# huster-wgm/SRCGAN

Measured on AMD Instinct MI355X. Metric: paired SR-CycleGAN train images/sec at x4 256->1024, higher is better.
Workload: dtype bf16; 1 GPU; Sat2Aerx4 paired G+D step (BASELINE configs[1]): 23-block RRDB generator + 3-layer PatchGAN, 3x256x256->3x1024x1024, batch 16/GPU; per_gpu_batch=16, global_batch=16, parallelism=dp1, gradient_exchange=none (1 rank)

## Files before the change

include/srcgan_amd.h:

```cpp
#ifndef SRCGAN_AMD_H
#define SRCGAN_AMD_H

#include <stddef.h>
#include <stdint.h>

#ifdef __cplusplus
extern "C" {
#endif

#define SRCGAN_F32 0
#define SRCGAN_BF16 1
#define SRCGAN_F16 2

int srcgan_version(void);
const char* srcgan_last_error(void);
int srcgan_dtype_size(int dtype);

int srcgan_nchw_f32_to_nhwc(const float* src, void* dst, int B, int C, int H, int W,
                            int cs, int dtype, void* stream);
int srcgan_nhwc_to_nchw_f32(const void* src, float* dst, int B, int C, int H, int W,
                            int cs, int coff, int dtype, void* stream);

size_t srcgan_packed_weight_bytes(int rows, int kdim, int ntaps, int dtype);
int srcgan_pack_weight(const float* w, void* wp, int rows, int kdim, int tys, int txs,
                       long sr, long sk, long sty, long stx, long off, int dtype, void* stream);
int srcgan_pack_weight_part(const float* w, void* wp, int rows, int kdim, int tys, int txs,
                            long sr, long sk, long sty, long stx, long off, int k_off, int k_total, float scale,
                            int dtype, void* stream);

typedef struct srcgan_conv_desc {
    const void* x; const void* wp; const float* bias; void* y;
    const void* r1; const void* r2; const void* mz;
    int dtype;
    int kh, kw, stride;
    int B, H, W, Cin, x_cs, x_coff;
    int OH, OW, Cout;
    int YH, YW, y_cs, y_coff;
    int pad_y, pad_x, os, oa, ob;
    int r1_cs, r1_coff, r1_cend;
    int r2_cs, r2_coff, r2_cend;
    int mz_cs, mz_coff, mz_c0;
    float alpha, beta1, beta2, slope, mslope;
    int act;
    long x_plane, y_plane, r1_plane, r2_plane, mz_plane;
    int rev_batch;
    void* sign_out; const void* sign_in;
    int npar; long wpar_stride;
} srcgan_conv_desc;
int srcgan_conv_igemm(const srcgan_conv_desc* d, void* stream);

typedef struct srcgan_wgrad_desc {
    const void* dy; const void* x; float* slab; float* grad;
    float* bias_grad;
    int dtype;
    int kh, kw, stride;
    int B, H, W, Cin, x_cs, x_coff;
    int OH, OW, Cout, dy_cs, dy_coff;
    int pad_y, pad_x;
    int nsplit;
    long sr, sk, sty, stx, off;
    float alpha;
    int accumulate;
} srcgan_wgrad_desc;
size_t srcgan_conv_wgrad_slab_bytes(int Cout, int Cin, int kh, int kw, int nsplit);
int srcgan_conv_wgrad_nsplit(int B, int OH, int OW, int Cout, int Cin, int stride);
int srcgan_conv_wgrad(const srcgan_wgrad_desc* d, void* stream);

typedef struct srcgan_wgrad_seg { int g0, g1; float* grad; float* bias; int Cin; float alpha; } srcgan_wgrad_seg;
typedef struct srcgan_wgrad_dense_desc {
    const void* dy; const void* x; float* slab;
    int dtype;
    int B, H, W;
    int G, dy_cs, dy_coff;
    int C, x_cs, x_coff;
    int nseg;
    srcgan_wgrad_seg seg[8];
    int accumulate;
    long dy_plane, x_plane;
} srcgan_wgrad_dense_desc;
size_t srcgan_wgrad_dense_slab_bytes(int G, int C, int dtype, int B, int H, int W);
int srcgan_wgrad_dense(const srcgan_wgrad_dense_desc* d, void* stream);

// ... 404 lines not shown
```

srcgan_amd/_native.py:

```python
from __future__ import annotations

import ctypes as C
import os
from typing import Optional, Sequence

import torch

_HERE = os.path.dirname(os.path.abspath(__file__))
LIB_PATH = os.environ.get("SRCGAN_AMD_LIB") or os.path.join(_HERE, "lib", "libsrcgan_amd.so")

F32, BF16, F16 = 0, 1, 2
_DTYPES = {"fp32": F32, "f32": F32, "float32": F32, torch.float32: F32,
           "bf16": BF16, "bfloat16": BF16, torch.bfloat16: BF16,
           "fp16": F16, "f16": F16, "float16": F16, "half": F16, torch.float16: F16, F32: F32, BF16: BF16, F16: F16}
_default_dtype = _DTYPES[os.environ.get("SRCGAN_AMD_DTYPE", "fp32")]


def dtype_id(d) -> int:
    if d is None:
        return _default_dtype
    try:
        return _DTYPES[d]
    except KeyError:
        raise ValueError(f"unsupported compute dtype {d!r} (use 'fp32', 'bf16' or 'fp16')") from None
# ... 88 lines not shown

class VdsrCfg(C.Structure):
    _fields_ = [(n, C.c_int) for n in ("in_ch", "B", "H", "W", "dtype", "n_resblocks", "n_feats")]


class ResnetGenCfg(C.Structure):
    _fields_ = [(n, C.c_int) for n in ("in_ch", "out_ch", "B", "H", "W", "dtype", "ngf", "n_blocks", "padding")]


class UnetCfg(C.Structure):
    _fields_ = [(n, C.c_int) for n in ("in_ch", "out_ch", "B", "H", "W", "dtype", "ngf", "num_downs")]


class VggLossCfg(C.Structure):
    _fields_ = [(n, C.c_int) for n in ("kind", "B", "H", "W", "dtype")]


class NLayerDCfg(C.Structure):
    _fields_ = [("in_ch", C.c_int), ("ndf", C.c_int), ("n_layers", C.c_int),
                ("B", C.c_int), ("H", C.c_int), ("W", C.c_int), ("dtype", C.c_int), ("training", C.c_int), ("norm", C.c_int)]


_P, _I, _L, _F, _S = C.c_void_p, C.c_int, C.c_long, C.c_float, C.c_size_t
SIGNATURES = {
    "srcgan_version": (_I, []),
    "srcgan_last_error": (C.c_char_p, []),
    "srcgan_dtype_size": (_I, [_I]),
    "srcgan_nchw_f32_to_nhwc": (_I, [_P, _P, _I, _I, _I, _I, _I, _I, _P]),
    "srcgan_nhwc_to_nchw_f32": (_I, [_P, _P, _I, _I, _I, _I, _I, _I, _I, _P]),
    "srcgan_packed_weight_bytes": (_S, [_I, _I, _I, _I]),
    "srcgan_pack_weight": (_I, [_P, _P, _I, _I, _I, _I, _L, _L, _L, _L, _L, _I, _P]),
    "srcgan_pack_weight_part": (_I, [_P, _P, _I, _I, _I, _I, _L, _L, _L, _L, _L, _I, _I, _F, _I, _P]),
    "srcgan_conv_igemm": (_I, [C.POINTER(ConvDesc), _P]),
    "srcgan_conv_wgrad_slab_bytes": (_S, [_I, _I, _I, _I, _I]),
    "srcgan_conv_wgrad_nsplit": (_I, [_I, _I, _I, _I, _I, _I]),
    "srcgan_conv_wgrad": (_I, [C.POINTER(WgradDesc), _P]),
    "srcgan_wgrad_dense_slab_bytes": (_S, [_I, _I, _I, _I, _I, _I]),
    "srcgan_wgrad_dense": (_I, [C.POINTER(WgradDenseDesc), _P]),
    "srcgan_col_reduce_blocks": (_I, [_L]),
    "srcgan_col_reduce": (_I, [_I, _P, _I, _I, _P, _I, _I, _P, _P, _L, _I, _F, _P, _P, _P, _I, _P]),
    "srcgan_bn_finalize": (_I, [_P, _P, _P, _P, _P, _P, _I, _L, _F, _F, _P]),
    "srcgan_bn_eval_rstd": (_I, [_P, _P, _I, _F, _P]),
    "srcgan_bn_apply_lrelu": (_I, [_P, _P, _P, _P, _P, _P, _L, _I, _I, _F, _I, _P]),
    "srcgan_bn_bwd_apply": (_I, [_P, _P, _P, _P, _P, _P, _P, _P, _L, _I, _I, _I, _P]),
    "srcgan_add_inplace": (_I, [_P, _I, _I, _P, _I, _I, _P, _I, _I, _F, _L, _I, _I, _P]),
    "srcgan_add_inplace_planes": (_I, [_P, _I, _I, _L, _P, _I, _I, _L, _P, _I, _I, _L, _F, _L, _I, _I, _P]),
    "srcgan_gn_scratch_floats": (_S, [_I, _I]),
    "srcgan_gn_forward": (_I, [_P, _I, _P, _I, _P, _I, _P, _P, _P, _I, _L, _I, _I, _F, _I, _F, _I, _P, _P]),
    "srcgan_gn_backward": (_I, [_P, _I, _P, _I, _P, _I, _P, _P, _P, _I, _P, _I, _I, _P, _P, _I, _F, _I, _L, _I, _I, _I, _P, _P]),
    "srcgan_ca_scratch_floats": (_S, [_I, _L, _I]),
    "srcgan_ca_forward": (_I, [_P, _I, _P, _I, _P, _I, _P, _P, _P, _P, _P, _I, _L, _I, _I, _I, _P, _P]),
    "srcgan_ca_backward": (_I, [_P, _I, _P, _I, _P, _P, _P, _P, _I, _P, _I, _I, _P, _P, _P, _P, _I, _L, _I, _I, _I, _P, _P]),
    "srcgan_s2d_shift": (_I, [_P, _I, _P, _I, _I, _I, _I, _I, _I, _I, _I, _I, _I, _P]),
    "srcgan_d2s_shift": (_I, [_P, _I, _P, _I, _I, _I, _I, _I, _I, _I, _I, _I, _I, _I, _P]),
    "srcgan_prelu_forward": (_I, [_P, _I, _P, _P, _P, _I, _F, _P, _I, _I, _I, _I, _I, _I, _I, _I, _I, _I, _P]),
    "srcgan_prelu_scratch_floats": (_S, [_I, _I, _I, _I, _I]),
    "srcgan_prelu_backward": (_I, [_P, _I, _P, _I, _P, _P, _P, _I, _P, _I, _F, _I, _P, _P, _I, _I, _I, _I, _I, _I, _I, _I, _I, _P, _P]),
    "srcgan_reflect_pad_nhwc": (_I, [_P, _I, _P, _I, _I, _I, _I, _I, _I, _I, _P]),
    "srcgan_reflect_pad_bwd_nhwc": (_I, [_P, _I, _P, _I, _I, _I, _I, _I, _I, _I, _I, _P]),
    "srcgan_tanh_forward": (_I, [_P, _I, _P, _I, _L, _I, _I, _P]),
    "srcgan_tanh_backward": (_I, [_P, _I, _P, _I, _P, _I, _L, _I, _I, _I, _P]),
    "srcgan_in_skip_forward": (_I, [_P, _I, _P, _I, _P, _I, _I, _P, _I, _L, _I, _F, _F, _I, _P, _P]),
    "srcgan_relu_nhwc": (_I, [_P, _I, _P, _I, _I, _L, _I, _I, _P]),
    "srcgan_upsample2_nhwc": (_I, [_P, _I, _I, _L, _P, _I, _I, _I, _I, _I, _I, _P]),
    "srcgan_sum2x2_nhwc": (_I, [_P, _I, _P, _I, _P, _I, _F, _I, _I, _I, _I, _I, _P]),
    "srcgan_loss_scratch_floats": (_I, []),
# ... 190 lines not shown
```

srcgan_amd/build.py:

```python
import glob
import os
import subprocess
import sys
from concurrent.futures import ThreadPoolExecutor

HERE = os.path.dirname(os.path.abspath(__file__))
CSRC = os.path.join(HERE, "csrc")
LIBDIR = os.path.join(HERE, "lib")
LIB = os.path.join(LIBDIR, "libsrcgan_amd.so")
SOURCES = ["conv_entry.hip", "conv_igemm.hip", "conv_par4.hip", "deconv_k3s2.hip", "conv3x3_dma.hip", "conv_wgrad.hip", "wgrad_dense.hip", "elementwise.hip", "class_losses.hip", "groupnorm.hip", "chan_attn.hip", "back_proj.hip", "reflect_pad.hip", "unet_skip.hip", "metrics.hip", "shift_select.hip", "scene_score.hip", "colour.hip", "tiles.hip", "vgg_loss.hip", "nets.hip", "oplist.hip"]
FLAGS = ["--offload-arch=gfx950", "-O3", "-std=c++17", "-fPIC", "-Wall", "-Wno-unused-function"]


def _hipcc():
    for c in (os.environ.get("HIPCC"), "/opt/rocm/bin/hipcc", "hipcc"):
        if c and (os.path.isabs(c) and os.path.exists(c) or not os.path.isabs(c)):
            return c
    raise RuntimeError("hipcc not found")


def _stale(target, deps):
    if not os.path.exists(target):
        return True
    t = os.path.getmtime(target)
    return any(os.path.getmtime(d) > t for d in deps)


def build(force=False, verbose=True):
    os.makedirs(LIBDIR, exist_ok=True)
    hipcc = _hipcc()
    headers = glob.glob(os.path.join(CSRC, "*.h")) + [os.path.join(HERE, "..", "include", "srcgan_amd.h")]
    objs, jobs = [], []
    for s in SOURCES:
        src = os.path.join(CSRC, s)
        obj = os.path.join(LIBDIR, s.replace(".hip", ".o"))
        objs.append(obj)
        if force or _stale(obj, [src] + headers):
            jobs.append([hipcc, *FLAGS, "-c", src, "-o", obj])

    def run(cmd):
        if verbose:
            print("[srcgan_amd.build]", " ".join(cmd), flush=True)
        subprocess.run(cmd, check=True)
# ... 13 lines not shown
```

srcgan_amd/csrc/conv_entry.hip:

```cpp
#include "conv_params.h"

static const bool g_force_generic = sg_env("SRCGAN_GENERIC_3X3") != nullptr;

static int check_desc(const srcgan_conv_desc* d) {
    SG_REQUIRE(d && d->x && d->wp && d->y, "srcgan_conv_igemm: null pointer");
    SG_REQUIRE(sg_dtype_ok(d->dtype), "srcgan_conv_igemm: bad dtype %d", d->dtype);
    const int epp = d->dtype == SRCGAN_F32 ? 4 : 8;
    SG_REQUIRE(d->B > 0 && d->H > 0 && d->W > 0 && d->OH > 0 && d->OW > 0 && d->Cin > 0 && d->Cout > 0,
               "srcgan_conv_igemm: non-positive dimension");
    SG_REQUIRE(d->Cin % epp == 0 && d->x_cs % epp == 0 && d->x_coff % epp == 0,
               "srcgan_conv_igemm: input channels/stride/offset (%d,%d,%d) must be multiples of %d", d->Cin, d->x_cs, d->x_coff, epp);
    SG_REQUIRE((d->x_plane || d->x_coff + d->Cin <= d->x_cs) && (d->y_plane || d->y_coff + d->Cout <= d->y_cs),
               "srcgan_conv_igemm: channel slice exceeds stride");
    SG_REQUIRE(!d->x_plane || (d->kh == 3 && d->kw == 3 && d->stride == 1), "srcgan_conv_igemm: a blocked-layout input is supported by the 3x3 stride-1 kernel only");
    SG_REQUIRE(((uintptr_t)d->x % 16) == 0 && ((uintptr_t)d->wp % 16) == 0, "srcgan_conv_igemm: x/wp must be 16-byte aligned");
    SG_REQUIRE(d->os >= 1 && d->oa >= 0 && d->ob >= 0 && d->oa < d->os && d->ob < d->os, "srcgan_conv_igemm: bad output scale/offset");
    SG_REQUIRE((d->OH - 1) * d->os + d->oa < d->YH && (d->OW - 1) * d->os + d->ob < d->YW, "srcgan_conv_igemm: output extent exceeds tensor");
    if (d->sign_out || d->sign_in) {
        const bool dense32 = d->kh == 3 && d->kw == 3 && d->stride == 1 && sg_is16(d->dtype) && d->Cout == 32 && d->os == 1 && d->oa == 0 && d->ob == 0 &&
                             d->YH == d->OH && d->YW == d->OW && d->x_plane && !(d->sign_in && d->mz) && (!d->sign_out || d->act);
        const bool up_out = d->sign_out && !d->sign_in && d->kh == 1 && d->kw == 1 && d->npar == 4 && sg_is16(d->dtype) && d->Cout == 64 && d->act;
        const bool in64 = d->sign_in && !d->sign_out && d->kh == 3 && d->kw == 3 && d->stride == 1 && sg_is16(d->dtype) && d->Cout == 64 && d->os == 1 &&
                          d->YH == d->OH && d->YW == d->OW && !d->mz && !d->r1 && !d->r2;
        SG_REQUIRE(dense32 || up_out || in64,
// ... 46 lines not shown
               "3x3 stride-1 form (pad 1, whole 64-byte input chunks, 18 rows below 2 GiB) takes larger images", p.H, p.W, p.xpix);
    return 0;
}

static int route(const srcgan_conv_desc* d, ConvP& p, hipStream_t st) {
    if (d->npar && d->kh == 3) {
        SG_REQUIRE(d->npar == 4 && d->kw == 3 && d->stride == 2 && d->pad_y == 1 && d->pad_x == 1 && d->os == 2 && d->oa == 0 && d->ob == 0 &&
                   d->OH == d->H && d->OW == d->W && d->YH == 2 * d->H && d->YW == 2 * d->W && d->wpar_stride > 0 && d->wpar_stride % 16 == 0 &&
                   !d->x_plane && !d->y_plane && !d->sign_in && !d->sign_out,
                   "srcgan_conv_igemm: npar == 4 with a 3x3 kernel is the transposed stride-2 form: stride 2, pad 1, os 2, oa == ob == 0, OH x OW = H x W, "
                   "YH x YW = 2H x 2W, the four parity packs wpar_stride bytes apart, interleaved tensors, no sign masks");
        SG_TRY(sg_require_image_31(p));
        p.npar = 4; p.wpar = d->wpar_stride;
        return sg_deconv_k3s2(p, d->dtype, st);
    }
    if (d->npar && d->kh == 1 && d->kw == 1) {
        SG_REQUIRE(d->npar == 4 && d->stride == 1 && d->os == 2 && d->oa == 0 && d->ob == 0 && d->wpar_stride > 0 && d->wpar_stride % 16 == 0 &&
                   !d->sign_in, "srcgan_conv_igemm: npar == 4 with a 1x1 kernel needs os == 2, oa == ob == 0 and the four packs wpar_stride bytes apart");
        SG_REQUIRE(!d->sign_out || p.buf16, "srcgan_conv_igemm: sign_out of the 1x1 four-parity form needs 16-byte accessible output channels");
        p.npar = 4; p.wpar = d->wpar_stride;
    } else if (d->npar) {
        SG_REQUIRE(d->npar == 4 && d->kh == 2 && d->kw == 2 && d->stride == 1 && d->wpar_stride > 0 && d->wpar_stride % 16 == 0 && !d->x_plane && !d->y_plane &&
                   !d->sign_in && !d->sign_out,
                   "srcgan_conv_igemm: npar must be 0 or 4 (2x2 stride-1 parity packs wpar_stride bytes apart, interleaved tensors, no bias / sign masks)");
        SG_TRY(sg_require_image_31(p));
        p.wpar = d->wpar_stride;
        return sg_dgrad_s2k4(p, d->dtype, st);
    }
    if (d->kh == 3 && d->kw == 3 && d->stride == 1 && (!g_force_generic || d->x_plane)) return sg_conv3x3_dma(p, d->dtype, st);
    SG_TRY(sg_require_image_31(p));
    return sg_conv_generic(p, d->dtype, d->kh, d->kw, d->stride, st);
}

extern "C" int srcgan_conv_igemm(const srcgan_conv_desc* d, void* stream) {
    SG_TRY(check_desc(d));
    ConvP p = build_params(d);
    return route(d, p, (hipStream_t)stream);
}
```

srcgan_amd/csrc/conv_igemm.hip:

```cpp
#include "conv_epilogue.h"
#include "launch.h"
#include <type_traits>

#if defined(SG_DIAG) && defined(SG_IG_DIAG)
#define IG_DBG(p, bit) ((p).dbg & (bit))
#else
#define IG_DBG(p, bit) 0
#endif


template <typename T, int KH, int KW, int S, int MT, int PT, bool WPK>
__global__ __launch_bounds__(256) void conv_igemm_k(const ConvP p) {
    using D = DT<T>;
    constexpr int TH = 4 * PT, TW = 32;
    constexpr int IHT = (TH - 1) * S + KH, IWT = (TW - 1) * S + KW;
    constexpr int COT = 32 * MT, NTAP = KH * KW, PIXB = 80;
    constexpr int WROWS = (WPK ? KW : NTAP) * COT;
    constexpr int NPH = IHT * IWT * 4;
    constexpr int NPW = WROWS * 4;
    constexpr int HIT = (NPH + 255) / 256, WIT = (NPW + 255) / 256;
    extern __shared__ __attribute__((aligned(16))) char smem[];
    char* lds_h = smem;
    char* lds_w = smem + IHT * IWT * PIXB;

// ... 253 lines not shown
#define SG_CASE(KH_, KW_, S_, PT_, WPK_) \
    if (kh == KH_ && kw == KW_ && s == S_) return launch_igemm<T, KH_, KW_, S_, MT, PT_, WPK_>(p, ctiles, st);
    SG_CASE(3, 3, 1, 2, false)
    SG_CASE(1, 1, 1, 2, false)
    SG_CASE(2, 2, 2, 1, false)
#ifndef SG_PT22
#define SG_PT22 2
#endif
    SG_CASE(2, 2, 1, SG_PT22, false)
    SG_CASE(1, 2, 1, 2, false)
    SG_CASE(2, 1, 1, 2, false)
    SG_CASE(4, 4, 2, 1, true)
    SG_CASE(4, 4, 1, 2, true)
    SG_CASE(3, 4, 1, 2, true)
    SG_CASE(4, 3, 1, 2, true)
    SG_CASE(3, 3, 2, 1, false)
    SG_CASE(7, 7, 2, 1, true)
    SG_CASE(1, 1, 2, 2, false)
    SG_CASE(5, 5, 1, 2, true)
    SG_CASE(9, 9, 1, 2, true)
    SG_CASE(7, 7, 1, 2, true)
#undef SG_CASE
    SG_FAIL("srcgan_conv_igemm: unsupported kernel %dx%d stride %d", kh, kw, s);
}

int sg_conv_generic(const ConvP& p, int dtype, int kh, int kw, int stride, hipStream_t st) {
    if (p.npar == 4 && kh == 1 && kw == 1 && sg_is16(dtype) && p.Cout == 64 && p.ypix == 128 && p.ycoff == 0 && p.yplane == 64 && p.YW == 2 * p.OW &&
        p.buf16 && !p.bias && !p.r1 && !p.r2 && !p.mz && p.Cin % 32 == 0) {
        ConvP q = p;
        q.npar = 2; q.wpar = 2 * p.wpar; q.wsplit = p.wpar;
        q.Cout = 128; q.ypix *= 2; q.YW = p.YW / 2; q.osx = 1;
        return sg_dtype_dispatch16(dtype, [&](auto t) { return launch_igemm<decltype(t), 1, 1, 1, 4, SG_UP_PT, false>(q, 2, st); });
    }
    const int npm = p.npar ? p.npar : 1;
    if (p.Cout <= 32) return sg_dtype_dispatch(dtype, [&](auto t) { return dispatch_shape<decltype(t), 1>(p, kh, kw, stride, npm, st); });
#ifdef SG_MT4_22
    if (dtype == SRCGAN_BF16 && kh == 2 && kw == 2 && stride == 1 && p.Cout % 128 == 0)
        return launch_igemm<__bf16, 2, 2, 1, 4, SG_PT22, false>(p, p.Cout / 128, st);
#endif
    const int ctiles = cdiv(p.Cout, 64) * npm;
    return sg_dtype_dispatch(dtype, [&](auto t) { return dispatch_shape<decltype(t), 2>(p, kh, kw, stride, ctiles, st); });
}
```

srcgan_amd/csrc/conv_par4.hip:

```cpp
#include "conv_epilogue.h"
#include "launch.h"
#include <type_traits>

template <typename T, int PT, bool VEC16>
__global__ __launch_bounds__(256, 2) void dgrad_s2k4_k(const ConvP p) {
    using D = DT<T>;
    constexpr int TH = 4 * PT, TW = 32, IHT = TH + 2, IWT = TW + 2;
    constexpr int COT = 32, PIXB = 80, NPAR = 4, WROWS = 16 * COT;
    constexpr int NPH = IHT * IWT * 4, NPW = WROWS * 4;
    constexpr int HIT = (NPH + 255) / 256, WIT = NPW / 256;
    static_assert(NPW % 256 == 0, "weight pieces per thread");
    extern __shared__ __attribute__((aligned(16))) char smem[];
    char* lds_h = smem;
    char* lds_w = smem + IHT * IWT * PIXB;

    const int tid = threadIdx.x, lane = tid & 63, wave = tid >> 6, r = lane & 31, h = lane >> 5;
    int L;
    {
        const int nblk = gridDim.x, bid = blockIdx.x, xcd = bid & 7, q8 = nblk >> 3, r8 = nblk & 7;
        L = (xcd < r8 ? xcd * (q8 + 1) : r8 * (q8 + 1) + (xcd - r8) * q8) + (bid >> 3);
    }
    const int ct = L % p.ctiles;
    int t = L / p.ctiles;
    const int tx = t % p.tiles_x; t /= p.tiles_x;
// ... 91 lines not shown
        pq.OH = (p.YH - pq.oa + 1) / 2; pq.OW = (p.YW - pq.ob + 1) / 2;
        if constexpr (VEC16) {
#pragma unroll
            for (int q = 0; q < PT; ++q) conv_epilogue_lds_row<T, 1, PT>(pq, acc[par], q, lw, b, ct, t0 + wave * PT + q, u0, lane);
        } else
            conv_epilogue<T, 1, PT>(pq, acc[par], b, ct, t0 + wave * PT, u0, r, h);
    }
}

template <typename T, int PT, bool VEC16>
static int launch_par4v(const ConvP& p, hipStream_t st) {
    constexpr int TH = 4 * PT, IHT = TH + 2, IWT = 34;
    constexpr size_t STAGE = (size_t)IHT * IWT * 80 + (size_t)16 * 32 * 80, EPI = (size_t)4 * 32 * (32 * 4 + 16);
    constexpr size_t SMEM = STAGE > EPI ? STAGE : EPI;
    constexpr auto kern = dgrad_s2k4_k<T, PT, VEC16>;
    int dev = 0;
    SG_TRY(sg_current_device(dev));
    SG_TRY(sg_allow_lds<kern>(SMEM, dev));
    ConvP q = p;
    q.tiles_x = cdiv((p.YW + 1) / 2, 32);
    q.tiles_y = cdiv((p.YH + 1) / 2, TH);
    q.ctiles = cdiv(p.Cout, 32);
    dim3 grid((unsigned)((size_t)q.tiles_x * q.tiles_y * p.B * q.ctiles), 1, 1);
    char cls[96];
    snprintf(cls, sizeof(cls), "dgrad_s2k4<%s,4 parities>", sg_dtype_tag<T>());
    const double px = (double)p.B * p.YH * p.YW;
    const int tok = sg_prof_start(cls, 2.0 * px * 4 * p.Cin * p.Cout, ((double)p.B * p.H * p.W * p.Cin + px * p.Cout) * sizeof(T), st);
    hipLaunchKernelGGL(kern, grid, dim3(256), SMEM, st, q);
    sg_prof_stop(tok, st);
    SG_LAUNCH_CHECK();
    return 0;
}

template <typename T, int PT>
static int launch_par4(const ConvP& p, hipStream_t st) {
    SG_REQUIRE(p.buf16, "srcgan_conv_igemm: npar == 4 needs output / mask channels, strides and offsets that are multiples of 16 bytes (and channel planes below 2 GiB)");
    return launch_par4v<T, PT, true>(p, st);
}

#ifndef SG_P4PT
#define SG_P4PT 2
#endif
int sg_dgrad_s2k4(const ConvP& p, int dtype, hipStream_t st) {
    return sg_dtype_dispatch(dtype, [&](auto t) { return launch_par4<decltype(t), SG_P4PT>(p, st); });
}
```

srcgan_amd/csrc/conv_params.h:

```cpp
#pragma once
#include "common.h"

struct ConvP {
    const void* x; const void* wp; const float* bias; void* y;
    const void* r1; const void* r2; const void* mz;
    int B, H, W, Cin, xcoff;
    int OH, OW, Cout, YH, YW, ycoff;
    int pad_y, pad_x, os, oa, ob;
    int r1coff, r1cend, r2coff, r2cend, mzcoff, mzc0;
    long xpix, xplane, ypix, yplane, r1pix, r1plane, r2pix, r2plane, mzpix, mzplane;
    float alpha, beta1, beta2, slope, mslope;
    int act, vec, nchunk, tiles_x, tiles_y, ctiles;
    int vec16;
    int buf16;
    int rev;
    long wpar;
    int npar;
    int osx;
    long wsplit;
    unsigned char* sgn_out; const unsigned char* sgn_in;
    int dbg;
    unsigned long long* trace;
};

template <typename T>
__device__ __forceinline__ size_t chan_off(int c, long plane) {
    constexpr int KCE = DT<T>::KCE;
    return (size_t)(c / KCE) * plane + (size_t)(c % KCE) * sizeof(T);
}

int sg_conv3x3_dma(const ConvP& p, int dtype, hipStream_t st);
int sg_dgrad_s2k4(const ConvP& p, int dtype, hipStream_t st);
int sg_deconv_k3s2(const ConvP& p, int dtype, hipStream_t st);
int sg_conv_generic(const ConvP& p, int dtype, int kh, int kw, int stride, hipStream_t st);
int sg_require_image_31(const ConvP& p);
```

srcgan_amd/ops.py:

```python
from __future__ import annotations

import ctypes as C
from typing import Optional, Tuple

import torch

from . import _native as N

TORCH_DT = {N.F32: torch.float32, N.BF16: torch.bfloat16, N.F16: torch.float16}


def to_nhwc(x: torch.Tensor, cs: Optional[int] = None, dtype=None) -> torch.Tensor:
    N.require_cuda(x, "to_nhwc")
    dt = N.dtype_id(dtype)
    x = x.contiguous().float()
    B, Cc, H, W = x.shape
    cs = cs or Cc
    out = torch.empty(B, H, W, cs, dtype=TORCH_DT[dt], device=x.device)
    N.check(N.lib().srcgan_nchw_f32_to_nhwc(x.data_ptr(), out.data_ptr(), B, Cc, H, W, cs, dt, N.stream_ptr(x.device)), "to_nhwc")
    return out


def to_nchw(x: torch.Tensor, Cc: Optional[int] = None, coff: int = 0) -> torch.Tensor:
    N.require_cuda(x, "to_nchw")
# ... 22 lines not shown
    return xb.permute(1, 2, 3, 0, 4).reshape(B, H, W, npl * kce)[..., :Cc].contiguous()


def pack_weight(w: torch.Tensor, rows: int, kdim: int, tys: int, txs: int, sr: int, sk: int, sty: int, stx: int,
                off: int = 0, dtype=None) -> torch.Tensor:
    N.require_cuda(w, "pack_weight")
    dt = N.dtype_id(dtype)
    lib = N.lib()
    nbytes = lib.srcgan_packed_weight_bytes(rows, kdim, tys * txs, dt)
    out = torch.empty(nbytes, dtype=torch.uint8, device=w.device)
    N.check(lib.srcgan_pack_weight(w.contiguous().data_ptr(), out.data_ptr(), rows, kdim, tys, txs, sr, sk, sty, stx, off, dt,
                                   N.stream_ptr(w.device)), "pack_weight")
    return out


def pack_conv2d_fwd(w: torch.Tensor, dtype=None) -> torch.Tensor:
    co, ci, kh, kw = w.shape
    return pack_weight(w, co, ci, kh, kw, ci * kh * kw, kh * kw, kw, 1, 0, dtype)


def pack_conv2d_dgrad_s1(w: torch.Tensor, dtype=None) -> torch.Tensor:
    co, ci, kh, kw = w.shape
    return pack_weight(w, ci, co, kh, kw, kh * kw, ci * kh * kw, -kw, -1, kh * kw - 1, dtype)


def conv_igemm(x: torch.Tensor, wp: torch.Tensor, y: torch.Tensor, *, kh: int, kw: int, stride: int = 1, Cin: Optional[int] = None,
               x_coff: int = 0, Cout: int, y_coff: int = 0, OH: Optional[int] = None, OW: Optional[int] = None,
               pad: Tuple[int, int] = (0, 0), bias: Optional[torch.Tensor] = None, alpha: float = 1.0, act: bool = False,
               slope: float = 0.2, r1: Optional[torch.Tensor] = None, r1_coff: int = 0, r1_cend: int = 0, beta1: float = 0.0,
               r2: Optional[torch.Tensor] = None, r2_coff: int = 0, r2_cend: int = 0, beta2: float = 0.0,
               mz: Optional[torch.Tensor] = None, mz_coff: int = 0, mz_c0: int = 0, mslope: float = 0.2,
               os: int = 1, oa: int = 0, ob: int = 0, x_plane: int = 0, y_plane: int = 0, r1_plane: int = 0, r2_plane: int = 0,
               mz_plane: int = 0, shape: Optional[Tuple[int, int, int]] = None, sign_out: Optional[torch.Tensor] = None,
               sign_in: Optional[torch.Tensor] = None, npar: int = 0, wpar_stride: int = 0, rev_batch: int = 0) -> torch.Tensor:
    N.require_cuda(x, "conv_igemm")
    d = N.ConvDesc()
    if shape is not None:
        (B, H, W), xcs = shape, x.shape[-1]
    else:
        B, H, W, xcs = x.shape
    d.x, d.wp, d.y = x.data_ptr(), wp.data_ptr(), y.data_ptr()
    d.bias = bias.data_ptr() if bias is not None else None
    d.dtype = N.dtype_id(x.dtype)
    d.kh, d.kw, d.stride = kh, kw, stride
    d.B, d.H, d.W, d.Cin, d.x_cs, d.x_coff = B, H, W, Cin or (xcs - x_coff), xcs, x_coff
    if OH is None:
        OH = (H + 2 * pad[0] - kh) // stride + 1
        OW = (W + 2 * pad[1] - kw) // stride + 1
    d.OH, d.OW, d.Cout = OH, OW, Cout
    d.YH, d.YW, d.y_cs, d.y_coff = (y.shape[-3], y.shape[-2], y.shape[-1], y_coff)
    d.pad_y, d.pad_x, d.os, d.oa, d.ob = pad[0], pad[1], os, oa, ob
    if r1 is not None:
        d.r1, d.r1_cs, d.r1_coff, d.r1_cend, d.beta1 = r1.data_ptr(), r1.shape[-1], r1_coff, r1_cend, beta1
    if r2 is not None:
        d.r2, d.r2_cs, d.r2_coff, d.r2_cend, d.beta2 = r2.data_ptr(), r2.shape[-1], r2_coff, r2_cend, beta2
    if mz is not None:
        d.mz, d.mz_cs, d.mz_coff, d.mz_c0 = mz.data_ptr(), mz.shape[-1], mz_coff, mz_c0
    if sign_out is not None:
        d.sign_out = sign_out.data_ptr()
    if sign_in is not None:
        d.sign_in = sign_in.data_ptr()
    d.npar, d.wpar_stride = npar, wpar_stride
    d.alpha, d.slope, d.mslope, d.act = alpha, slope, mslope, int(act)
    d.x_plane, d.y_plane, d.r1_plane, d.r2_plane, d.mz_plane = x_plane, y_plane, r1_plane, r2_plane, mz_plane
    d.rev_batch = rev_batch
    N.check(N.lib().srcgan_conv_igemm(C.byref(d), N.stream_ptr(x.device)), "srcgan_conv_igemm")
    return y


def pack_deconv3x3s2(w: torch.Tensor, dtype=None):
    N.require_cuda(w, "pack_deconv3x3s2")
    lib = N.lib()
    dt = N.dtype_id(dtype)
    cin, cout = w.shape[:2]
    w = w.contiguous().float()
    step = lib.srcgan_packed_weight_bytes(cout, cin, 4, dt)
    wp = torch.zeros(4 * step, dtype=torch.uint8, device=w.device)
    for q in range(4):
        a, b = q >> 1, q & 1
        N.check(lib.srcgan_pack_weight(w.data_ptr(), wp.data_ptr() + q * step, cout, cin, a + 1, b + 1, 9, cout * 9, -6, -2,
                                       (2 if a else 1) * 3 + (2 if b else 1), dt, N.stream_ptr(w.device)), "srcgan_pack_weight")
    return wp, step


def deconv3x3s2(x: torch.Tensor, w: torch.Tensor, bias: Optional[torch.Tensor] = None, relu: bool = False, packed=None,
                y: Optional[torch.Tensor] = None) -> torch.Tensor:
    N.require_cuda(x, "deconv3x3s2")
    B, H, W, _ = x.shape
    cout = w.shape[1]
    wp, step = packed if packed is not None else pack_deconv3x3s2(w, x.dtype)
    if y is None:
        y = torch.empty(B, 2 * H, 2 * W, cout, dtype=x.dtype, device=x.device)
    return conv_igemm(x, wp, y, kh=3, kw=3, stride=2, Cout=cout, OH=H, OW=W, pad=(1, 1), bias=bias, act=relu, slope=0.0, os=2,
                      npar=4, wpar_stride=step)


def conv_wgrad(dy: torch.Tensor, x: torch.Tensor, grad: torch.Tensor, *, kh: int, kw: int, stride: int = 1, Cout: int, Cin: int,
               dy_coff: int = 0, x_coff: int = 0, pad: Tuple[int, int] = (0, 0), layout: Tuple[int, int, int, int, int],
               alpha: float = 1.0, nsplit: Optional[int] = None, accumulate: bool = False,
               bias_grad: Optional[torch.Tensor] = None) -> torch.Tensor:
# ... 158 lines not shown
```

Baseline: 120.3 images/s.

## Add LDS-staged tiled kernels for 4x4 stride-2 conv and its parity dgrad

Adds a new persistent kernel for 4x4 stride-2 pad-1 convolutions in 16-bit types. It stages an 8x32 output tile's input halo and weights into LDS using async global-to-LDS loads with double buffering, and uses XCD-aware work distribution. It also adds a similar tiled kernel for the 4-parity 2x2 dgrad (the transpose of the stride-2 conv) that reuses one 3x3 input window across all parities. Both are meant to replace the generic igemm path for the PatchGAN downsampling layers and their backward passes, improving data reuse and overlapping loads with MFMA. A path-query API is added so callers can see which kernel a descriptor selects.

```diff
diff --git a/include/srcgan_amd.h b/include/srcgan_amd.h
--- a/include/srcgan_amd.h
+++ b/include/srcgan_amd.h
@@ -48,6 +48,7 @@
     int npar; long wpar_stride;
 } srcgan_conv_desc;
 int srcgan_conv_igemm(const srcgan_conv_desc* d, void* stream);
+int srcgan_conv_path(const srcgan_conv_desc* d);
 
 typedef struct srcgan_wgrad_desc {
     const void* dy; const void* x; float* slab; float* grad;
diff --git a/srcgan_amd/_native.py b/srcgan_amd/_native.py
--- a/srcgan_amd/_native.py
+++ b/srcgan_amd/_native.py
@@ -144,6 +144,7 @@
     "srcgan_pack_weight": (_I, [_P, _P, _I, _I, _I, _I, _L, _L, _L, _L, _L, _I, _P]),
     "srcgan_pack_weight_part": (_I, [_P, _P, _I, _I, _I, _I, _L, _L, _L, _L, _L, _I, _I, _F, _I, _P]),
     "srcgan_conv_igemm": (_I, [C.POINTER(ConvDesc), _P]),
+    "srcgan_conv_path": (_I, [C.POINTER(ConvDesc)]),
     "srcgan_conv_wgrad_slab_bytes": (_S, [_I, _I, _I, _I, _I]),
     "srcgan_conv_wgrad_nsplit": (_I, [_I, _I, _I, _I, _I, _I]),
     "srcgan_conv_wgrad": (_I, [C.POINTER(WgradDesc), _P]),
diff --git a/srcgan_amd/build.py b/srcgan_amd/build.py
--- a/srcgan_amd/build.py
+++ b/srcgan_amd/build.py
@@ -8,7 +8,7 @@
 CSRC = os.path.join(HERE, "csrc")
 LIBDIR = os.path.join(HERE, "lib")
 LIB = os.path.join(LIBDIR, "libsrcgan_amd.so")
-SOURCES = ["conv_entry.hip", "conv_igemm.hip", "conv_par4.hip", "deconv_k3s2.hip", "conv3x3_dma.hip", "conv_wgrad.hip", "wgrad_dense.hip", "elementwise.hip", "class_losses.hip", "groupnorm.hip", "chan_attn.hip", "back_proj.hip", "reflect_pad.hip", "unet_skip.hip", "metrics.hip", "shift_select.hip", "scene_score.hip", "colour.hip", "tiles.hip", "vgg_loss.hip", "nets.hip", "oplist.hip"]
+SOURCES = ["conv_entry.hip", "conv_igemm.hip", "conv_s2_tile8.hip", "conv_par4.hip", "deconv_k3s2.hip", "conv3x3_dma.hip", "conv_wgrad.hip", "wgrad_dense.hip", "elementwise.hip", "class_losses.hip", "groupnorm.hip", "chan_attn.hip", "back_proj.hip", "reflect_pad.hip", "unet_skip.hip", "metrics.hip", "shift_select.hip", "scene_score.hip", "colour.hip", "tiles.hip", "vgg_loss.hip", "nets.hip", "oplist.hip"]
 FLAGS = ["--offload-arch=gfx950", "-O3", "-std=c++17", "-fPIC", "-Wall", "-Wno-unused-function"]
 
 
diff --git a/srcgan_amd/csrc/conv_entry.hip b/srcgan_amd/csrc/conv_entry.hip
--- a/srcgan_amd/csrc/conv_entry.hip
+++ b/srcgan_amd/csrc/conv_entry.hip
@@ -102,6 +102,16 @@
     return sg_conv_generic(p, d->dtype, d->kh, d->kw, d->stride, st);
 }
 
+extern "C" int srcgan_conv_path(const srcgan_conv_desc* d) {
+    if (check_desc(d)) return -1;
+    const ConvP p = build_params(d);
+    if (d->npar == 4 && d->kh == 2 && d->kw == 2 && d->stride == 1 && d->wpar_stride > 0 && d->wpar_stride % 16 == 0 && !d->x_plane && !d->y_plane &&
+        !d->sign_in && !d->sign_out)
+        return sg_dgrad_s2k4_tile64_ok(p, d->dtype) ? 2 : 0;
+    const bool generic = !d->npar && !(d->kh == 3 && d->kw == 3 && d->stride == 1);
+    return generic && sg_conv_s2_tile8_ok(p, d->dtype, d->kh, d->kw, d->stride) ? 1 : 0;
+}
+
 extern "C" int srcgan_conv_igemm(const srcgan_conv_desc* d, void* stream) {
     SG_TRY(check_desc(d));
     ConvP p = build_params(d);
diff --git a/srcgan_amd/csrc/conv_igemm.hip b/srcgan_amd/csrc/conv_igemm.hip
--- a/srcgan_amd/csrc/conv_igemm.hip
+++ b/srcgan_amd/csrc/conv_igemm.hip
@@ -309,6 +309,7 @@
         q.Cout = 128; q.ypix *= 2; q.YW = p.YW / 2; q.osx = 1;
         return sg_dtype_dispatch16(dtype, [&](auto t) { return launch_igemm<decltype(t), 1, 1, 1, 4, SG_UP_PT, false>(q, 2, st); });
     }
+    if (sg_conv_s2_tile8_ok(p, dtype, kh, kw, stride)) return sg_conv_s2_tile8(p, dtype, st);
     const int npm = p.npar ? p.npar : 1;
     if (p.Cout <= 32) return sg_dtype_dispatch(dtype, [&](auto t) { return dispatch_shape<decltype(t), 1>(p, kh, kw, stride, npm, st); });
 #ifdef SG_MT4_22
diff --git a/srcgan_amd/csrc/conv_par4.hip b/srcgan_amd/csrc/conv_par4.hip
--- a/srcgan_amd/csrc/conv_par4.hip
+++ b/srcgan_amd/csrc/conv_par4.hip
@@ -147,6 +147,164 @@
     return 0;
 }
 
+static __device__ __attribute__((aligned(64))) unsigned int sg_p4_zero_page[16];
+typedef const __attribute__((address_space(1))) void* p4_gptr_t;
+typedef __attribute__((address_space(3))) void* p4_lptr_t;
+
+namespace p4t {
+constexpr int NWV = 8, TH = 8, TW = 32, IHT = TH + 2, IWT = TW + 2, COT = 64, REC = 32;
+constexpr int NHP = IHT * IWT;
+constexpr int HPIECES = (NHP * REC + 1023) / 1024, WPIECES = 16 * COT * REC / 1024;
+constexpr int HBYTES = HPIECES * 1024, WBYTES = WPIECES * 1024, SBYTES = HBYTES + WBYTES;
+constexpr int HIT = (HPIECES + NWV - 1) / NWV, WIT = WPIECES / NWV;
+constexpr int ERS = 32 * 4 + 16;
+constexpr size_t SMEM = 2 * (size_t)SBYTES;
+static_assert(WIT == 4, "weight piece `it` of a wave belongs to parity `it`: 8 pieces = 256 records per parity");
+static_assert(NWV * 32 * ERS <= SBYTES, "epilogue transpose space must fit one stage");
+__device__ __forceinline__ int half_off(int rec, int half) { return (half ^ ((rec >> 3) & 1)) * 16; }
+}
+
+template <typename T>
+__global__ __launch_bounds__(p4t::NWV * 64) void dgrad_s2k4_tile64_k(const ConvP p) {
+    using namespace p4t;
+    extern __shared__ __attribute__((aligned(1024))) char smem[];
+    const int tid = threadIdx.x, lane = tid & 63, r = lane & 31, h = lane >> 5;
+    const int wave = __builtin_amdgcn_readfirstlane(tid >> 6);
+    const int rp = wave & 3, mt = wave >> 2;
+    const int nunits = p.tiles_x * p.tiles_y * p.B * p.ctiles;
+    const int xcd = blockIdx.x & 7, jw = blockIdx.x >> 3, gw = (gridDim.x + 7 - xcd) >> 3;
+    const int u8 = (nunits + 7) >> 3;
+    const int u_lo = xcd * u8, u_hi = (u_lo + u8 < nunits) ? u_lo + u8 : nunits;
+    const char* zp = (const char*)sg_p4_zero_page;
+    const int nhalf = 2 * p.nchunk;
+
+    int w_off[WIT];
+#pragma unroll
+    for (int it = 0; it < WIT; ++it) {
+        const int q = (it * NWV + wave) * 64 + lane, rec = q >> 1;
+        w_off[it] = (rec & 255) * 64 + half_off(rec, q & 1);
+    }
+    int h_goff[HIT];
+    const char* f_xb = nullptr; const char* f_wb = nullptr;
+    auto setup_fetch = [&](int u, int& ob, int& oct, int& ot0, int& ou0) {
+        const int ct = u % p.ctiles; int t = u / p.ctiles;
+        const int tx = t % p.tiles_x; t /= p.tiles_x;
+        const int ty = t % p.tiles_y; const int b = t / p.tiles_y;
+        ob = b; oct = ct; ot0 = ty * TH; ou0 = tx * TW;
+        f_xb = (const char*)p.x + (size_t)b * p.H * p.W * p.xpix + (size_t)p.xcoff * sizeof(T);
+        f_wb = (const char*)p.wp + (size_t)ct * p.nchunk * 4 * COT * 64;
+#pragma unroll
+        for (int it = 0; it < HIT; ++it) {
+            const int q = (it * NWV + wave) * 64 + lane, rec = q >> 1;
+            const int iy = rec / IWT, ix = rec - iy * IWT;
+            const int gy = ot0 - 1 + iy, gx = ou0 - 1 + ix;
+            const bool ok = rec < NHP && (unsigned)gy < (unsigned)p.H && (unsigned)gx < (unsigned)p.W;
+            h_goff[it] = ok ? (gy * p.W + gx) * (int)p.xpix + half_off(rec, q & 1) : -1;
+        }
+    };
+    auto issue = [&](int s, int stage) {
+        char* lh = smem + stage * SBYTES;
+        char* lw = lh + HBYTES;
+#pragma unroll
+        for (int it = 0; it < HIT; ++it) {
+            const int pi = it * NWV + wave;
+            if (HIT * NWV == HPIECES || pi < HPIECES) {
+                const char* src = h_goff[it] >= 0 ? f_xb + h_goff[it] + s * REC : zp;
+                __builtin_amdgcn_global_load_lds((p4_gptr_t)src, (p4_lptr_t)(lh + pi * 1024), 16, 0, 0);
+            }
+        }
+        const char* ws = f_wb + (size_t)(s >> 1) * 4 * COT * 64 + (s & 1) * REC;
+#pragma unroll
+        for (int it = 0; it < WIT; ++it)
+            __builtin_amdgcn_global_load_lds((p4_gptr_t)(ws + (size_t)it * p.wpar + w_off[it]), (p4_lptr_t)(lw + (it * NWV + wave) * 1024), 16, 0, 0);
+    };
+
+    int u = u_lo + jw;
+    if (u >= u_hi) return;
+    int cb, cct, ct0, cu0, nb_, nct, nt0, nu0;
+    setup_fetch(u, nb_, nct, nt0, nu0);
+    issue(0, 0);
+    int stage = 0;
+    for (; u < u_hi; u += gw) {
+        cb = nb_; cct = nct; ct0 = nt0; cu0 = nu0;
+        f32x16 acc[4][1][2];
+#pragma unroll
+        for (int q = 0; q < 4; ++q)
+#pragma unroll
+            for (int k = 0; k < 2; ++k)
+#pragma unroll
+                for (int i = 0; i < 16; ++i) acc[q][0][k][i] = 0.f;
+
+        for (int s = 0; s < nhalf; ++s, stage ^= 1) {
+            asm volatile("s_waitcnt vmcnt(0)" ::: "memory");
+            __syncthreads();
+            if (s + 1 < nhalf) issue(s + 1, stage ^ 1);
+            else if (u + gw < u_hi) { setup_fetch(u + gw, nb_, nct, nt0, nu0); issue(0, stage ^ 1); }
+            const char* lh = smem + stage * SBYTES;
+            const char* lw = lh + HBYTES;
+#pragma unroll
+            for (int wy = 0; wy < 3; ++wy)
+#pragma unroll
+                for (int wx = 0; wx < 3; ++wx) {
+                    bf16x8 bb[2];
+#pragma unroll
+                    for (int q = 0; q < 2; ++q) {
+                        const int rec = (rp * 2 + q + wy) * IWT + r + wx;
+                        bb[q] = *(const bf16x8*)(lh + rec * REC + half_off(rec, h));
+                    }
+#pragma unroll
+                    for (int par = 0; par < 4; ++par) {
+                        const int tyy = wy - (par >> 1), txx = wx - (par & 1);
+                        if (tyy < 0 || tyy > 1 || txx < 0 || txx > 1) continue;
+                        const int rec = (par * 4 + tyy * 2 + txx) * COT + mt * 32 + r;
+                        const bf16x8 a = *(const bf16x8*)(lw + rec * REC + half_off(rec, h));
+#pragma unroll
+                        for (int q = 0; q < 2; ++q) acc[par][0][q] = sg_mfma16<T>(a, bb[q], acc[par][0][q]);
+                    }
+                }
+        }
+        __syncthreads();
+        char* lwv = smem + (stage ^ 1) * SBYTES + wave * (32 * ERS);
+#pragma unroll
+        for (int par = 0; par < 4; ++par) {
+            ConvP pq = p;
+            pq.os = 2; pq.oa = par >> 1; pq.ob = par & 1;
+            pq.OH = (p.YH - pq.oa + 1) / 2; pq.OW = (p.YW - pq.ob + 1) / 2;
+#pragma unroll
+            for (int q = 0; q < 2; ++q) conv_epilogue_lds_row<T, 1, 2>(pq, acc[par], q, lwv, cb, cct * 2 + mt, ct0 + rp * 2 + q, cu0, lane);
+        }
+    }
+}
+
+bool sg_dgrad_s2k4_tile64_ok(const ConvP& p, int dtype) {
+    using namespace p4t;
+    return sg_is16(dtype) && p.buf16 && p.xplane == 64 && p.Cin % 32 == 0 && p.Cout % COT == 0 && p.YH % (2 * TH) == 0 && p.YW % (2 * TW) == 0 &&
+           p.H == p.YH / 2 && p.W == p.YW / 2 && !p.sgn_in && !p.sgn_out && (long)p.B * (p.H / TH) * (p.W / TW) * (p.Cout / COT) < (1L << 30);
+}
+
+template <typename T>
+static int launch_par4_tile64(const ConvP& p, hipStream_t st) {
+    using namespace p4t;
+    constexpr auto kern = dgrad_s2k4_tile64_k<T>;
+    int dev = 0;
+    SG_TRY(sg_current_device(dev));
+    SG_TRY(sg_allow_lds<kern>(SMEM, dev));
+    const int ncu = sg_cu_count(dev);
+    if (!ncu) return 1;
+    ConvP q = p;
+    q.tiles_x = p.W / TW; q.tiles_y = p.H / TH; q.ctiles = p.Cout / COT;
+    const size_t nunits = (size_t)q.tiles_x * q.tiles_y * p.B * q.ctiles;
+    const size_t nwg = nunits < (size_t)ncu ? nunits : (size_t)ncu;
+    char cls[96];
+    snprintf(cls, sizeof(cls), "dgrad_s2k4<%s,4 parities>", sg_dtype_tag<T>());
+    const double px = (double)p.B * p.YH * p.YW;
+    const int tok = sg_prof_start(cls, 2.0 * px * 4 * p.Cin * p.Cout, ((double)p.B * p.H * p.W * p.Cin + px * p.Cout) * sizeof(T), st);
+    hipLaunchKernelGGL(kern, dim3((unsigned)nwg), dim3(NWV * 64), SMEM, st, q);
+    sg_prof_stop(tok, st);
+    SG_LAUNCH_CHECK();
+    return 0;
+}
+
 template <typename T, int PT>
 static int launch_par4(const ConvP& p, hipStream_t st) {
     SG_REQUIRE(p.buf16, "srcgan_conv_igemm: npar == 4 needs output / mask channels, strides and offsets that are multiples of 16 bytes (and channel planes below 2 GiB)");
@@ -157,5 +315,6 @@
 #define SG_P4PT 2
 #endif
 int sg_dgrad_s2k4(const ConvP& p, int dtype, hipStream_t st) {
+    if (sg_dgrad_s2k4_tile64_ok(p, dtype)) return sg_dtype_dispatch16(dtype, [&](auto t) { return launch_par4_tile64<decltype(t)>(p, st); });
     return sg_dtype_dispatch(dtype, [&](auto t) { return launch_par4<decltype(t), SG_P4PT>(p, st); });
 }
diff --git a/srcgan_amd/csrc/conv_params.h b/srcgan_amd/csrc/conv_params.h
--- a/srcgan_amd/csrc/conv_params.h
+++ b/srcgan_amd/csrc/conv_params.h
@@ -31,6 +31,9 @@
 
 int sg_conv3x3_dma(const ConvP& p, int dtype, hipStream_t st);
 int sg_dgrad_s2k4(const ConvP& p, int dtype, hipStream_t st);
+bool sg_dgrad_s2k4_tile64_ok(const ConvP& p, int dtype);
 int sg_deconv_k3s2(const ConvP& p, int dtype, hipStream_t st);
 int sg_conv_generic(const ConvP& p, int dtype, int kh, int kw, int stride, hipStream_t st);
+bool sg_conv_s2_tile8_ok(const ConvP& p, int dtype, int kh, int kw, int stride);
+int sg_conv_s2_tile8(const ConvP& p, int dtype, hipStream_t st);
 int sg_require_image_31(const ConvP& p);
diff --git a/srcgan_amd/csrc/conv_s2_tile8.hip b/srcgan_amd/csrc/conv_s2_tile8.hip
--- /dev/null
+++ b/srcgan_amd/csrc/conv_s2_tile8.hip
@@ -0,0 +1,159 @@
+#include "conv_epilogue.h"
+#include "launch.h"
+
+static __device__ __attribute__((aligned(64))) unsigned int sg_s2_zero_page[16];
+
+typedef const __attribute__((address_space(1))) void* s2_gptr_t;
+typedef __attribute__((address_space(3))) void* s2_lptr_t;
+
+namespace {
+constexpr int NWV = 8, TH = 8, TW = 32, IHT = 2 * TH + 2, IWT = 2 * TW + 2, IWH = IWT / 2;
+constexpr int COT = 64, NTAP = 16, REC = 32;
+constexpr int NHP = IHT * IWT;
+constexpr int HPIECES = (NHP * REC + 1023) / 1024;
+constexpr int WPIECES = NTAP * COT * REC / 1024;
+constexpr int HBYTES = HPIECES * 1024, WBYTES = WPIECES * 1024, SBYTES = HBYTES + WBYTES;
+constexpr int HIT = (HPIECES + NWV - 1) / NWV, WIT = WPIECES / NWV;
+constexpr int ERS = COT * 4 + 16;
+constexpr size_t SMEM = 2 * (size_t)SBYTES;
+static_assert(WPIECES % NWV == 0, "weight pieces per wave");
+static_assert(NWV * 32 * ERS <= SBYTES, "epilogue transpose space must fit one stage");
+static_assert(SMEM <= 160 * 1024, "LDS budget");
+}
+
+__device__ __forceinline__ int s2_half(int rec, int half) { return (half ^ ((rec >> 3) & 1)) * 16; }
+
+template <typename T>
+__global__ __launch_bounds__(NWV * 64) void conv4x4s2_tile8_k(const ConvP p) {
+    extern __shared__ __attribute__((aligned(1024))) char smem[];
+    const int tid = threadIdx.x, lane = tid & 63, r = lane & 31, h = lane >> 5;
+    const int wave = __builtin_amdgcn_readfirstlane(tid >> 6);
+    const int nunits = p.tiles_x * p.tiles_y * p.B * p.ctiles;
+    const int xcd = blockIdx.x & 7, jw = blockIdx.x >> 3, gw = (gridDim.x + 7 - xcd) >> 3;
+    const int u8 = (nunits + 7) >> 3;
+    const int u_lo = xcd * u8, u_hi = (u_lo + u8 < nunits) ? u_lo + u8 : nunits;
+    const char* zp = (const char*)sg_s2_zero_page;
+    const int nhalf = 2 * p.nchunk;
+
+    int w_off[WIT];
+#pragma unroll
+    for (int it = 0; it < WIT; ++it) {
+        const int q = (it * NWV + wave) * 64 + lane, rec = q >> 1;
+        w_off[it] = rec * 64 + s2_half(rec, q & 1);
+    }
+    int h_goff[HIT];
+    const char* f_xb = nullptr; const char* f_wb = nullptr;
+    auto setup_fetch = [&](int u, int& ob, int& oct, int& ooy0, int& oox0) {
+        const int ct = u % p.ctiles; int t = u / p.ctiles;
+        const int tx = t % p.tiles_x; t /= p.tiles_x;
+        const int ty = t % p.tiles_y; const int b = t / p.tiles_y;
+        ob = b; oct = ct; ooy0 = ty * TH; oox0 = tx * TW;
+        const int gy0 = ooy0 * 2 - 1, gx0 = oox0 * 2 - 1;
+        f_xb = (const char*)p.x + (size_t)b * p.H * p.W * p.xpix + (size_t)p.xcoff * sizeof(T);
+        f_wb = (const char*)p.wp + (size_t)ct * p.nchunk * NTAP * COT * 64;
+#pragma unroll
+        for (int it = 0; it < HIT; ++it) {
+            const int q = (it * NWV + wave) * 64 + lane, rec = q >> 1;
+            const int iy = rec / IWT, lx = rec - iy * IWT;
+            const int ix = lx < IWH ? 2 * lx : 2 * (lx - IWH) + 1;
+            const int gy = gy0 + iy, gx = gx0 + ix;
+            const bool ok = rec < NHP && (unsigned)gy < (unsigned)p.H && (unsigned)gx < (unsigned)p.W;
+            h_goff[it] = ok ? (gy * p.W + gx) * (int)p.xpix + s2_half(rec, q & 1) : -1;
+        }
+    };
+    auto issue = [&](int s, int stage) {
+        char* lh = smem + stage * SBYTES;
+        char* lw = lh + HBYTES;
+#pragma unroll
+        for (int it = 0; it < HIT; ++it) {
+            const int pi = it * NWV + wave;
+            if (HIT * NWV == HPIECES || pi < HPIECES) {
+                const char* src = h_goff[it] >= 0 ? f_xb + h_goff[it] + s * REC : zp;
+                __builtin_amdgcn_global_load_lds((s2_gptr_t)src, (s2_lptr_t)(lh + pi * 1024), 16, 0, 0);
+            }
+        }
+        const char* ws = f_wb + (size_t)(s >> 1) * NTAP * COT * 64 + (s & 1) * REC;
+#pragma unroll
+        for (int it = 0; it < WIT; ++it)
+            __builtin_amdgcn_global_load_lds((s2_gptr_t)(ws + w_off[it]), (s2_lptr_t)(lw + (it * NWV + wave) * 1024), 16, 0, 0);
+    };
+
+    int u = u_lo + jw;
+    if (u >= u_hi) return;
+    int cb, cct, coy0, cox0;
+    int nb_, nct, noy0, nox0;
+    setup_fetch(u, nb_, nct, noy0, nox0);
+    issue(0, 0);
+    int stage = 0;
+    for (; u < u_hi; u += gw) {
+        cb = nb_; cct = nct; coy0 = noy0; cox0 = nox0;
+        f32x16 acc[2][1];
+#pragma unroll
+        for (int m = 0; m < 2; ++m)
+#pragma unroll
+            for (int i = 0; i < 16; ++i) acc[m][0][i] = 0.f;
+
+        for (int s = 0; s < nhalf; ++s, stage ^= 1) {
+            asm volatile("s_waitcnt vmcnt(0)" ::: "memory");
+            __syncthreads();
+            if (s + 1 < nhalf) issue(s + 1, stage ^ 1);
+            else if (u + gw < u_hi) { setup_fetch(u + gw, nb_, nct, noy0, nox0); issue(0, stage ^ 1); }
+            const char* lh = smem + stage * SBYTES;
+            const char* lw = lh + HBYTES;
+            bf16x8 fa[2][2], fb[2];
+            auto load_step = [&](int tap, bf16x8 (&a)[2], bf16x8& bq) {
+                const int ky = tap >> 2, kx = tap & 3;
+#pragma unroll
+                for (int m = 0; m < 2; ++m) {
+                    const int rec = tap * COT + m * 32 + r;
+                    a[m] = *(const bf16x8*)(lw + rec * REC + s2_half(rec, h));
+                }
+                const int rec = (2 * wave + ky) * IWT + (kx & 1) * IWH + (kx >> 1) + r;
+                bq = *(const bf16x8*)(lh + rec * REC + s2_half(rec, h));
+            };
+            load_step(0, fa[0], fb[0]);
+#pragma unroll
+            for (int tap = 0; tap < NTAP; ++tap) {
+                if (tap + 1 < NTAP) load_step(tap + 1, fa[(tap + 1) & 1], fb[(tap + 1) & 1]);
+                __builtin_amdgcn_sched_barrier(0);
+#pragma unroll
+                for (int m = 0; m < 2; ++m) acc[m][0] = sg_mfma16<T>(fa[tap & 1][m], fb[tap & 1], acc[m][0]);
+                __builtin_amdgcn_sched_barrier(0);
+            }
+        }
+        __syncthreads();
+        conv_epilogue_lds_row<T, 2, 1>(p, acc, 0, smem + (stage ^ 1) * SBYTES + wave * (32 * ERS), cb, cct, coy0 + wave, cox0, lane);
+    }
+}
+
+bool sg_conv_s2_tile8_ok(const ConvP& p, int dtype, int kh, int kw, int stride) {
+    return sg_is16(dtype) && kh == 4 && kw == 4 && stride == 2 && !p.npar && p.pad_y == 1 && p.pad_x == 1 && p.Cin % 32 == 0 && p.Cout % COT == 0 &&
+           p.OH % TH == 0 && p.OW % TW == 0 && p.H == 2 * p.OH && p.W == 2 * p.OW && p.buf16 && p.xplane == 64 && !p.sgn_in && !p.sgn_out &&
+           (long)p.B * (p.OH / TH) * (p.OW / TW) * (p.Cout / COT) < (1L << 30);
+}
+
+template <typename T>
+static int launch_s2_tile8(const ConvP& p, hipStream_t st) {
+    constexpr auto kern = conv4x4s2_tile8_k<T>;
+    int dev = 0;
+    SG_TRY(sg_current_device(dev));
+    SG_TRY(sg_allow_lds<kern>(SMEM, dev));
+    const int ncu = sg_cu_count(dev);
+    if (!ncu) return 1;
+    ConvP q = p;
+    q.tiles_x = p.OW / TW; q.tiles_y = p.OH / TH; q.ctiles = p.Cout / COT;
+    const size_t nunits = (size_t)q.tiles_x * q.tiles_y * p.B * q.ctiles;
+    const size_t nwg = nunits < (size_t)ncu ? nunits : (size_t)ncu;
+    char cls[96];
+    snprintf(cls, sizeof(cls), "conv_igemm<%s,4x4,s2,MT2>", sg_dtype_tag<T>());
+    const double px = (double)p.B * p.OH * p.OW;
+    const int tok = sg_prof_start(cls, 2.0 * px * NTAP * p.Cin * p.Cout, ((double)p.B * p.H * p.W * p.Cin + px * p.Cout) * sizeof(T), st);
+    hipLaunchKernelGGL(kern, dim3((unsigned)nwg), dim3(NWV * 64), SMEM, st, q);
+    sg_prof_stop(tok, st);
+    SG_LAUNCH_CHECK();
+    return 0;
+}
+
+int sg_conv_s2_tile8(const ConvP& p, int dtype, hipStream_t st) {
+    return sg_dtype_dispatch16(dtype, [&](auto t) { return launch_s2_tile8<decltype(t)>(p, st); });
+}
diff --git a/srcgan_amd/ops.py b/srcgan_amd/ops.py
--- a/srcgan_amd/ops.py
+++ b/srcgan_amd/ops.py
@@ -78,7 +78,7 @@
                mz: Optional[torch.Tensor] = None, mz_coff: int = 0, mz_c0: int = 0, mslope: float = 0.2,
                os: int = 1, oa: int = 0, ob: int = 0, x_plane: int = 0, y_plane: int = 0, r1_plane: int = 0, r2_plane: int = 0,
                mz_plane: int = 0, shape: Optional[Tuple[int, int, int]] = None, sign_out: Optional[torch.Tensor] = None,
-               sign_in: Optional[torch.Tensor] = None, npar: int = 0, wpar_stride: int = 0, rev_batch: int = 0) -> torch.Tensor:
+               sign_in: Optional[torch.Tensor] = None, npar: int = 0, wpar_stride: int = 0, rev_batch: int = 0, path_only: bool = False) -> torch.Tensor:
     N.require_cuda(x, "conv_igemm")
     d = N.ConvDesc()
     if shape is not None:
@@ -110,8 +110,14 @@
     d.alpha, d.slope, d.mslope, d.act = alpha, slope, mslope, int(act)
     d.x_plane, d.y_plane, d.r1_plane, d.r2_plane, d.mz_plane = x_plane, y_plane, r1_plane, r2_plane, mz_plane
     d.rev_batch = rev_batch
+    if path_only:
+        return N.lib().srcgan_conv_path(C.byref(d))
     N.check(N.lib().srcgan_conv_igemm(C.byref(d), N.stream_ptr(x.device)), "srcgan_conv_igemm")
     return y
+
+
+def conv_path(x: torch.Tensor, wp: torch.Tensor, y: torch.Tensor, **kw) -> int:
+    return conv_igemm(x, wp, y, path_only=True, **kw)
 
 
 def pack_deconv3x3s2(w: torch.Tensor, dtype=None):
```

Result: no change. 120.3 images/s, median of 6 (+0.0%).
